# mcahny/vps

Hardware: AMD Instinct MI355X
Metric: frames/sec FuseTrack 1024x2048 (higher is better)
Workload: dtype f32-grade: f16x3 split operands (fp16 pair with scaled residual, 22 significand bits) on MFMA, f32 accumulate

## Files before the change

### vps_amd/csrc/conv_h8.hip

```cpp
#include "conv_common.h"

namespace {

template <int MODE, int KH, int KW>
__global__ __launch_bounds__(512, 2)
void conv_mfma_h8_kernel(const vps_conv_desc d, const int tiles_m, const int tiles_n, const int chunks_per_split) {
    constexpr int TM = 2, TN = 2, WAVES_N = 2, BN = 128;
    constexpr int NTAP = KH * KW;
    constexpr int HW = 32 + KW - 1, HH = 8 + KH - 1;
    constexpr int HROWS = HH * HW;
    constexpr int NLD = (HROWS + 63) / 64;
    typedef Split<MODE> SM;
    typedef typename SM::elem elem_t;
    typedef vec8<elem_t> x8;
    typedef vec4<elem_t> x4;
    constexpr int NSA = SM::NSA, NSB = SM::NSB;
    constexpr int PLANE = NLD * 64 * LDS_LDH;
    constexpr int ABUF = NSA * PLANE;
    constexpr int NLB = NSB;
    constexpr int NFRAG = NLB * 2 * (BN / 32);
    constexpr int BBUF = NFRAG * 512;
    static_assert((NFRAG * 64) % 512 == 0, "whole 16-byte chunks per thread");
    constexpr int NBL = NFRAG * 64 / 512;
    static_assert(2 * (ABUF + BBUF) * 2 <= 160 * 1024, "LDS budget of the CU");

    __shared__ __attribute__((aligned(16))) elem_t As[2 * ABUF];
    __shared__ __attribute__((aligned(16))) elem_t Bs[2 * BBUF];

    const int t = threadIdx.x;
    int swz = xcd_swizzle(blockIdx.x, gridDim.x);
    int tile_n, tile_m, cls, split;
    decode_tile(d, swz, tiles_n, tiles_m, tile_n, tile_m, cls, split);

    const int py = cls / d.os_x, px = cls - py * d.os_x;
    const int H = d.H, W = d.W, cin_pad = d.cin_pad;
    const int tiles_x = (d.Qw + 31) >> 5, tiles_y = (d.Qh + 7) >> 3;
    const int tx = tile_m % tiles_x, tq = tile_m / tiles_x;
    const int ty = tq % tiles_y, n = tq / tiles_y;
    const int iy_org = ty * 8 - d.pad_y[py], ix_org = tx * 32 - d.pad_x[px];

    const int k4 = t & 7;
    const int r0 = t >> 3;
    const int chunk0 = split * chunks_per_split;
    const int nchunks = min(chunks_per_split, d.kpad / (BK * NTAP) - chunk0);
    const int nsteps = nchunks * NTAP;

    const int lane = t & 63;
    const int wave = __builtin_amdgcn_readfirstlane(t >> 6);
    const int wm = wave / WAVES_N, wn = wave - wm * WAVES_N;
    const int nbt = d.cout_pad >> 5, kst = d.kpad >> 4;
    const size_t wplane = (size_t)d.nclass * nbt * kst * 512;
    const __amdgpu_buffer_rsrc_t wrsrc = make_rsrc(d.w_split, (unsigned)(wplane * NSB * sizeof(elem_t)));
    const unsigned wbase = (unsigned)((((size_t)(cls * nbt + tile_n * (BN / 32)) * kst + 2 * (size_t)chunk0 * NTAP) * 512) * sizeof(elem_t));
    const __amdgpu_buffer_rsrc_t arsrc = make_rsrc(d.in, (unsigned)((size_t)d.N * H * W * d.in_ld * sizeof(float)));
    const unsigned ld4 = (unsigned)d.in_ld * 4u;

    f32x4 areg[NLD];
    int achunk = chunk0;
    x8 breg[NBL];
    float amax = 0.f;

    unsigned hoff[NLD];
#pragma unroll
    for (int i = 0; i < NLD; ++i) {
        const int hp = r0 + 64 * i;
        const int hy = hp / HW, hx = hp - hy * HW;
        const int iy = iy_org + hy, ix = ix_org + hx;
        const bool ok = hp < HROWS && (unsigned)iy < (unsigned)H && (unsigned)ix < (unsigned)W;
        hoff[i] = ok ? (unsigned)((n * H + iy) * W + ix) * ld4 + (unsigned)(d.in_coff + k4 * 4) * 4u : 0xFFFFFFF0u;
    }

    auto load_A = [&]() {
        const bool kv = achunk * BK + k4 * 4 < cin_pad;
        const unsigned coff = (unsigned)achunk * (BK * 4u);
        ++achunk;
#pragma unroll
        for (int i = 0; i < NLD; ++i)
            areg[i] = buffer_load16<f32x4>(arsrc, (kv && hoff[i] != 0xFFFFFFF0u) ? hoff[i] + coff : 0xFFFFFFF0u, 0u);
    };
    auto store_A = [&](int i, int buf) {
        x4 sp[NSA];
        split_act<MODE>(areg[i], sp, amax);
        const int row = r0 + 64 * i;
#pragma unroll
        for (int p = 0; p < NSA; ++p)
            *reinterpret_cast<x4*>(&As[buf * ABUF + p * PLANE + row * LDS_LDH + (((k4 >> 1) ^ lds_swz(row)) << 3) + ((k4 & 1) << 2)]) = sp[p];
    };
    auto load_B = [&](int step) {
#pragma unroll
        for (int j = 0; j < NBL; ++j) {
            const int f = __builtin_amdgcn_readfirstlane((t + 512 * j) >> 6), bcol = f % (BN / 32), pm = f / (BN / 32);
            breg[j] = buffer_load16<x8>(wrsrc, (unsigned)lane * 16u,
                                        wbase + (unsigned)(((size_t)(pm >> 1) * wplane + ((size_t)bcol * kst + 2 * step + (pm & 1)) * 512) * sizeof(elem_t)));
        }
    };
    auto store_B = [&](int buf) {
#pragma unroll
        for (int j = 0; j < NBL; ++j) *reinterpret_cast<x8*>(&Bs[buf * BBUF + (t + 512 * j) * 8]) = breg[j];
    };

    int hbase[TM];
#pragma unroll
    for (int a = 0; a < TM; ++a) hbase[a] = (wm * TM + a) * HW + (lane & 31);
    x8 af[2][NSA][TM];
    auto read_A = [&](int m, int buf, int toff) {
#pragma unroll
        for (int a = 0; a < TM; ++a) {
            const int hrow = hbase[a] + toff;
            const int off = buf * ABUF + hrow * LDS_LDH + (((2 * m + (lane >> 5)) ^ lds_swz(hrow)) << 3);
#pragma unroll
            for (int p = 0; p < NSA; ++p) af[m][p][a] = *reinterpret_cast<const x8*>(&As[off + p * PLANE]);
        }
    };
    x8 bcur[2][NSB][TN];
    auto read_B = [&](int m, int buf) {
#pragma unroll
        for (int p = 0; p < NLB; ++p)
#pragma unroll
            for (int b = 0; b < TN; ++b)
                bcur[m][p][b] = *reinterpret_cast<const x8*>(&Bs[buf * BBUF + (((p * 2 + m) * (BN / 32)) + wn * TN + b) * 512 + lane * 8]);
        if constexpr (NLB < NSB) {
#pragma unroll
            for (int b = 0; b < TN; ++b) bcur[m][2][b] = derive_weight_plane<MODE>(bcur[m][0][b]);
        }
    };

    f32x16 acc[TM][TN];
#pragma unroll
    for (int a = 0; a < TM; ++a)
#pragma unroll
        for (int b = 0; b < TN; ++b)
#pragma unroll
            for (int r = 0; r < 16; ++r) acc[a][b][r] = 0.f;

    load_A();
    load_B(0);
#pragma unroll
    for (int i = 0; i < NLD; ++i) store_A(i, 0);
    store_B(0);
    load_A();
    __syncthreads();

    constexpr int NT = SM::NT;
    constexpr int NMF = 2 * NT * TM * TN;
    constexpr int SPT = (NLD + NTAP - 2) / (NTAP - 1);
    constexpr int NW = SPT + 3;

    for (int chunk = 0; chunk < nchunks; ++chunk) {
        const int cur = chunk & 1;
#pragma unroll
        for (int tp = 0; tp < NTAP; ++tp) {
            const int step = chunk * NTAP + tp;
            const int bb = step & 1;
            const int bstep = min(step + 1, nsteps - 1);
            const int toff = (tp / KW) * HW + (tp % KW);
            read_A(0, cur, toff);
            read_B(0, bb);
            __builtin_amdgcn_sched_barrier(0);

            auto work = [&](const int w) {
                if (w == 0) load_B(bstep);
                else if (w == 1) { read_A(1, cur, toff); read_B(1, bb); }
                else if (w < SPT + 2) {
                    const int si = w - 2;
                    if (tp < NTAP - 1) {
                        const int row = tp * SPT + si;
                        if (row < NLD) store_A(row, cur ^ 1);
                    } else if (si == 0) load_A();
                } else store_B(bb ^ 1);
            };

            int mf = 0;
#pragma unroll
            for (int m = 0; m < 2; ++m)
#pragma unroll
                for (int q = 0; q < NT; ++q)
#pragma unroll
                    for (int a = 0; a < TM; ++a)
#pragma unroll
                        for (int b = 0; b < TN; ++b) {
                            acc[a][b] = split_mfma<MODE>(bcur[m][SM::PB[q]][b], af[m][SM::PA[q]][a], acc[a][b]);
                            ++mf;
#pragma unroll
                            for (int w = 0; w < NW; ++w) {
                                const int pos = ((w + 1) * NMF) / (NW + 1);
                                if (mf == (pos < 1 ? 1 : pos)) {
                                    __builtin_amdgcn_sched_barrier(0);
                                    work(w);
                                    __builtin_amdgcn_sched_barrier(0);
                                }
                            }
                        }
            __syncthreads();
        }
    }
    report_range<MODE>(d, amax);
    conv_epilogue<TM, TN, BN, true, 5>(d, acc, tiles_m * 256, tile_m, tile_n, cls, split, py, px, wm, wn, lane, (cls * tiles_m + tile_m) * tiles_n + tile_n);
}

struct S2Tap { int ph, j, i, idx, t, nt; };
constexpr int s2_taps_1d(int K, int a) { return (K - a + 1) / 2; }
constexpr S2Tap s2_tap(int K, int ts) {
    int base = 0;
    for (int ph = 0; ph < 4; ++ph) {
        const int a = ph >> 1, b = ph & 1, J = s2_taps_1d(K, a), I = s2_taps_1d(K, b);
        if (ts < base + J * I) {
            const int t = ts - base, j = t / I, i = t - j * I;
            return S2Tap{ph, j, i, (2 * j + a) * K + 2 * i + b, t, J * I};
        }
        base += J * I;
    }
    return S2Tap{0, 0, 0, 0, 0, 1};
}
template <int N, typename F>
__device__ __forceinline__ void static_for(F&& f) {
    if constexpr (N > 0) {
        static_for<N - 1>(f);
        f(std::integral_constant<int, N - 1>{});
    }
}

template <int MODE, int K, int BN = 128>
__global__ __launch_bounds__(512, 2)
void conv_mfma_h8s2_kernel(const vps_conv_desc d, const int tiles_m, const int tiles_n, const int chunks_per_split) {
    static_assert(BN == 128 || BN == 64, "two column waves of 64 or 32 columns");
    constexpr int TM = 2, TN = BN / 64, WAVES_N = 2;
    constexpr int NTAP = K * K;
    constexpr int J0 = s2_taps_1d(K, 0);
    constexpr int HW = 32 + J0 - 1, HH = 8 + J0 - 1;
    constexpr int HROWS = HH * HW;
    constexpr int NLD = (HROWS + 63) / 64;
    typedef Split<MODE> SM;
    typedef typename SM::elem elem_t;
    typedef vec8<elem_t> x8;
    typedef vec4<elem_t> x4;
    constexpr int NSA = SM::NSA, NSB = SM::NSB;
    constexpr int PLANE = NLD * 64 * LDS_LDH;
    constexpr int ABUF = NSA * PLANE;
    constexpr int NLB = NSB;
    constexpr int NFRAG = NLB * 2 * (BN / 32);
    constexpr int NBL = (NFRAG * 64 + 511) / 512;
    constexpr bool WHOLE = (NFRAG * 64) % 512 == 0;
    constexpr int BBUF = NBL * 512 * 8;
    static_assert(2 * (ABUF + BBUF) * 2 <= 160 * 1024, "LDS budget of the CU");

    __shared__ __attribute__((aligned(16))) elem_t As[2 * ABUF];
    __shared__ __attribute__((aligned(16))) elem_t Bs[2 * BBUF];

    const int t = threadIdx.x;
    const int swz = xcd_swizzle(blockIdx.x, gridDim.x);
    int tile_n, tile_m, cls, split;
    decode_tile(d, swz, tiles_n, tiles_m, tile_n, tile_m, cls, split);

    const int H = d.H, W = d.W, cin_pad = d.cin_pad;
    const int tiles_x = (d.Qw + 31) >> 5, tiles_y = (d.Qh + 7) >> 3;
    const int tx = tile_m % tiles_x, tq = tile_m / tiles_x;
    const int ty = tq % tiles_y, n = tq / tiles_y;
    const int iy_org = ty * 16 - d.pad_y[0], ix_org = tx * 64 - d.pad_x[0];

    const int k4 = t & 7;
    const int r0 = t >> 3;
    const int chunk0 = split * chunks_per_split;
    const int nchunks = min(chunks_per_split, d.kpad / (BK * NTAP) - chunk0);

    const int lane = t & 63;
    const int wave = __builtin_amdgcn_readfirstlane(t >> 6);
    const int wm = wave / WAVES_N, wn = wave - wm * WAVES_N;
    const int nbt = d.cout_pad >> 5, kst = d.kpad >> 4;
    const size_t wplane = (size_t)nbt * kst * 512;
    const __amdgpu_buffer_rsrc_t wrsrc = make_rsrc(d.w_split, (unsigned)(wplane * NSB * sizeof(elem_t)));
    const unsigned wbase = (unsigned)((((size_t)(tile_n * (BN / 32)) * kst + 2 * (size_t)chunk0 * NTAP) * 512) * sizeof(elem_t));
    const __amdgpu_buffer_rsrc_t arsrc = make_rsrc(d.in, (unsigned)((size_t)d.N * H * W * d.in_ld * sizeof(float)));
    const unsigned ld4 = (unsigned)d.in_ld * 4u;

    f32x4 areg[NLD];
    int achunk = chunk0, aph = 0;
    x8 breg[NBL];
    float amax = 0.f;

    auto load_A = [&]() {
        const int a = aph >> 1, b = aph & 1;
        const int rows = 8 + ((K - a + 1) >> 1) - 1, cols = 32 + ((K - b + 1) >> 1) - 1;
        const int cic = achunk * BK + k4 * 4;
        const bool kv = cic < cin_pad;
        const unsigned coff = (unsigned)(d.in_coff + cic) * 4u;
        if (++aph == 4) { aph = 0; ++achunk; }
#pragma unroll
        for (int i = 0; i < NLD; ++i) {
            const int hp = r0 + 64 * i;
            const int hy = hp / HW, hx = hp - hy * HW;
            const int iy = iy_org + a + 2 * hy, ix = ix_org + b + 2 * hx;
            const bool ok = kv && hy < rows && hx < cols && (unsigned)iy < (unsigned)H && (unsigned)ix < (unsigned)W;
            areg[i] = buffer_load16<f32x4>(arsrc, ok ? (unsigned)((n * H + iy) * W + ix) * ld4 + coff : 0xFFFFFFF0u, 0u);
        }
    };
    auto store_A = [&](int i, int buf) {
        x4 sp[NSA];
        split_act<MODE>(areg[i], sp, amax);
        const int row = r0 + 64 * i;
#pragma unroll
        for (int p = 0; p < NSA; ++p)
            *reinterpret_cast<x4*>(&As[buf * ABUF + p * PLANE + row * LDS_LDH + (((k4 >> 1) ^ lds_swz(row)) << 3) + ((k4 & 1) << 2)]) = sp[p];
    };
    auto load_B = [&](int wstep) {
#pragma unroll
        for (int j = 0; j < NBL; ++j) {
            const int fr = __builtin_amdgcn_readfirstlane((t + 512 * j) >> 6), f = WHOLE ? fr : min(fr, NFRAG - 1);
            const int bcol = f % (BN / 32), pm = f / (BN / 32);
            breg[j] = buffer_load16<x8>(wrsrc, (unsigned)lane * 16u,
                                        wbase + (unsigned)(((size_t)(pm >> 1) * wplane + ((size_t)bcol * kst + 2 * wstep + (pm & 1)) * 512) * sizeof(elem_t)));
        }
    };
    auto store_B = [&](int buf) {
#pragma unroll
        for (int j = 0; j < NBL; ++j)
            *reinterpret_cast<x8*>(&Bs[buf * BBUF + (t + 512 * j) * 8]) = breg[j];
    };

    int hbase[TM];
#pragma unroll
    for (int a = 0; a < TM; ++a) hbase[a] = (wm * TM + a) * HW + (lane & 31);
    x8 af[2][NSA][TM];
    auto read_A = [&](int m, int buf, int toff) {
#pragma unroll
        for (int a = 0; a < TM; ++a) {
            const int hrow = hbase[a] + toff;
            const int off = buf * ABUF + hrow * LDS_LDH + (((2 * m + (lane >> 5)) ^ lds_swz(hrow)) << 3);
#pragma unroll
            for (int p = 0; p < NSA; ++p) af[m][p][a] = *reinterpret_cast<const x8*>(&As[off + p * PLANE]);
        }
    };
    x8 bcur[2][NSB][TN];
    auto read_B = [&](int m, int buf) {
#pragma unroll
        for (int p = 0; p < NLB; ++p)
#pragma unroll
            for (int b = 0; b < TN; ++b)
                bcur[m][p][b] = *reinterpret_cast<const x8*>(&Bs[buf * BBUF + (((p * 2 + m) * (BN / 32)) + wn * TN + b) * 512 + lane * 8]);
        if constexpr (NLB < NSB) {
#pragma unroll
            for (int b = 0; b < TN; ++b) bcur[m][2][b] = derive_weight_plane<MODE>(bcur[m][0][b]);
        }
    };

    f32x16 acc[TM][TN];
#pragma unroll
    for (int a = 0; a < TM; ++a)
#pragma unroll
        for (int b = 0; b < TN; ++b)
#pragma unroll
            for (int r = 0; r < 16; ++r) acc[a][b][r] = 0.f;

    load_A();
    load_B(s2_tap(K, 0).idx);
#pragma unroll
    for (int i = 0; i < NLD; ++i) store_A(i, 0);
    store_B(0);
    load_A();
    __syncthreads();

    constexpr int NT = SM::NT;
    constexpr int NMF = 2 * NT * TM * TN;

    for (int chunk = 0; chunk < nchunks; ++chunk) {
        static_for<NTAP>([&](auto ts_tag) {
            constexpr int TS = decltype(ts_tag)::value;
            constexpr S2Tap tp = s2_tap(K, TS);
            constexpr S2Tap nx = s2_tap(K, (TS + 1) % NTAP);
            constexpr int cur = tp.ph & 1;
            constexpr bool last_of_phase = tp.t == tp.nt - 1;
            constexpr int SPT = (NLD + tp.nt - 1) / tp.nt;
            constexpr int NW = 3 + SPT + (last_of_phase ? 1 : 0);
            const int step = chunk * NTAP + TS;
            const int bb = step & 1;
            const int wnext = (TS + 1 < NTAP ? chunk : min(chunk + 1, nchunks - 1)) * NTAP + nx.idx;
            constexpr int toff = tp.j * HW + tp.i;
            read_A(0, cur, toff);
            read_B(0, bb);
            __builtin_amdgcn_sched_barrier(0);

            auto work = [&](const int w) {
                if (w == 0) load_B(wnext);
                else if (w == 1) { read_A(1, cur, toff); read_B(1, bb); }
                else if (w < SPT + 2) {
                    const int row = tp.t * SPT + (w - 2);
                    if (row < NLD) store_A(row, cur ^ 1);
                } else if (last_of_phase && w == SPT + 2) load_A();
                else store_B(bb ^ 1);
            };

            int mf = 0;
#pragma unroll
            for (int m = 0; m < 2; ++m)
#pragma unroll
                for (int q = 0; q < NT; ++q)
#pragma unroll
                    for (int a = 0; a < TM; ++a)
#pragma unroll
                        for (int b = 0; b < TN; ++b) {
                            acc[a][b] = split_mfma<MODE>(bcur[m][SM::PB[q]][b], af[m][SM::PA[q]][a], acc[a][b]);
                            ++mf;
#pragma unroll
                            for (int w = 0; w < NW; ++w) {
                                const int pos = ((w + 1) * NMF) / (NW + 1);
                                if (mf == (pos < 1 ? 1 : pos)) {
                                    __builtin_amdgcn_sched_barrier(0);
                                    work(w);
                                    __builtin_amdgcn_sched_barrier(0);
                                }
                            }
                        }
            __syncthreads();
        });
    }
    report_range<MODE>(d, amax);
    conv_epilogue<TM, TN, BN, true, 5>(d, acc, tiles_m * 256, tile_m, tile_n, cls, split, 0, 0, wm, wn, lane, (cls * tiles_m + tile_m) * tiles_n + tile_n);
}

}

int vpsi_launch_conv_h8p(const vps_conv_desc& d, int tiles_m8, int tiles_n, int chunks_per_split, long nblk8, hipStream_t s);

__attribute__((visibility("hidden")))
void vpsi_launch_conv_h8(const vps_conv_desc& d, int tiles_m8, int tiles_n, int chunks_per_split, long nblk8, hipStream_t s) {
    if (vpsi_launch_conv_h8p(d, tiles_m8, tiles_n, chunks_per_split, nblk8, s)) return;
#define VPS_H8_LAUNCH(MODE, K)                                                                                                   \
    hipLaunchKernelGGL((conv_mfma_h8_kernel<MODE, K, K>), dim3((unsigned)nblk8), dim3(512), 0, s, d, tiles_m8, tiles_n, chunks_per_split)
    if (d.prec == VPS_PREC_BF16) { if (d.KH == 3) VPS_H8_LAUNCH(VPS_PREC_BF16, 3); else VPS_H8_LAUNCH(VPS_PREC_BF16, 2); }
    else if (d.prec == VPS_PREC_BF16X3) { if (d.KH == 3) VPS_H8_LAUNCH(VPS_PREC_BF16X3, 3); else VPS_H8_LAUNCH(VPS_PREC_BF16X3, 2); }
    else { if (d.KH == 3) VPS_H8_LAUNCH(VPS_PREC_F16X3, 3); else VPS_H8_LAUNCH(VPS_PREC_F16X3, 2); }
#undef VPS_H8_LAUNCH
}

__attribute__((visibility("hidden")))
void vpsi_launch_conv_h8s2(const vps_conv_desc& d, int tiles_m8, int tiles_n, int chunks_per_split, long nblk8, int bn, hipStream_t s) {
#define VPS_H8S2_LAUNCH(MODE, K)                                                                                                 \
    do {                                                                                                                         \
        if (bn == 64) hipLaunchKernelGGL((conv_mfma_h8s2_kernel<MODE, K, 64>), dim3((unsigned)nblk8), dim3(512), 0, s, d, tiles_m8, tiles_n, chunks_per_split); \
        else hipLaunchKernelGGL((conv_mfma_h8s2_kernel<MODE, K, 128>), dim3((unsigned)nblk8), dim3(512), 0, s, d, tiles_m8, tiles_n, chunks_per_split);         \
    } while (0)
    if (d.prec == VPS_PREC_BF16) { if (d.KH == 3) VPS_H8S2_LAUNCH(VPS_PREC_BF16, 3); else VPS_H8S2_LAUNCH(VPS_PREC_BF16, 5); }
    else if (d.prec == VPS_PREC_BF16X3) { if (d.KH == 3) VPS_H8S2_LAUNCH(VPS_PREC_BF16X3, 3); else VPS_H8S2_LAUNCH(VPS_PREC_BF16X3, 5); }
    else { if (d.KH == 3) VPS_H8S2_LAUNCH(VPS_PREC_F16X3, 3); else VPS_H8S2_LAUNCH(VPS_PREC_F16X3, 5); }
#undef VPS_H8S2_LAUNCH
}
```

Before: 56.47.

## Add wide-N 3x3 f16x3 conv kernel with register-staged activations

Adds a new conv kernel for 3x3 f16x3 convolutions with cout divisible by 256. It uses a 256-wide N tile with a 2x4 wave layout and TM=4, so each activation halo tile is reused across twice as many output channels. Activations are loaded into registers early and written into the second LDS buffer across the first taps, weights are DMA'd directly into LDS with buffer_load_lds, and the third weight plane is derived in registers rather than stored. The kernel is used by default when its shape conditions hold, can be turned off with VPS_H8W=0, and raises register and LDS pressure per block.

Result: faster. 57.06, median of 6 (+1.1%).

```diff
diff --git a/vps_amd/csrc/conv_h8.hip b/vps_amd/csrc/conv_h8.hip
--- a/vps_amd/csrc/conv_h8.hip
+++ b/vps_amd/csrc/conv_h8.hip
@@ -420,9 +420,11 @@
 }
 
 int vpsi_launch_conv_h8p(const vps_conv_desc& d, int tiles_m8, int tiles_n, int chunks_per_split, long nblk8, hipStream_t s);
+int vpsi_launch_conv_h8w(const vps_conv_desc& d, int tiles_m8, int chunks_per_split, hipStream_t s);
 
 __attribute__((visibility("hidden")))
 void vpsi_launch_conv_h8(const vps_conv_desc& d, int tiles_m8, int tiles_n, int chunks_per_split, long nblk8, hipStream_t s) {
+    if (vpsi_launch_conv_h8w(d, tiles_m8, chunks_per_split, s)) return;
     if (vpsi_launch_conv_h8p(d, tiles_m8, tiles_n, chunks_per_split, nblk8, s)) return;
 #define VPS_H8_LAUNCH(MODE, K)                                                                                                   \
     hipLaunchKernelGGL((conv_mfma_h8_kernel<MODE, K, K>), dim3((unsigned)nblk8), dim3(512), 0, s, d, tiles_m8, tiles_n, chunks_per_split)
diff --git a/vps_amd/csrc/conv_h8w.hip b/vps_amd/csrc/conv_h8w.hip
--- /dev/null
+++ b/vps_amd/csrc/conv_h8w.hip
@@ -0,0 +1,231 @@
+#include "conv_common.h"
+
+namespace {
+
+template <int N, typename F>
+__device__ __forceinline__ void static_for_w(F&& f) {
+    if constexpr (N > 0) {
+        static_for_w<N - 1>(f);
+        f(std::integral_constant<int, N - 1>{});
+    }
+}
+
+template <int N>
+__device__ __forceinline__ void wait_vm_lgkm0() {
+    static_assert(N >= 0 && N < 64, "vmcnt range");
+    asm volatile("s_waitcnt vmcnt(%0) lgkmcnt(0)" ::"n"(N) : "memory");
+}
+
+__global__ __launch_bounds__(512, 2)
+void conv_mfma_h8w_kernel(const vps_conv_desc d, const int tiles_m, const int tiles_n, const int chunks_per_split) {
+    constexpr int MODE = VPS_PREC_F16X3;
+    constexpr int KH = 3, KW = 3;
+    constexpr int TM = 4, TN = 2, WAVES_N = 4, BN = 256;
+    constexpr int NTAP = KH * KW;
+    constexpr int HW = 32 + KW - 1, HH = 8 + KH - 1;
+    constexpr int HROWS = HH * HW;
+    constexpr int NLD = (HROWS + 63) / 64;
+    typedef Split<MODE> SM;
+    typedef typename SM::elem elem_t;
+    typedef vec8<elem_t> x8;
+    typedef vec4<elem_t> x4;
+    constexpr int NSA = SM::NSA, NLB = SM::NLB;
+    static_assert(NSA == 2 && NLB == 2 && SM::NSB == 3 && SM::NT == 3, "f16x3: two activation planes, two stored weight planes");
+    constexpr int PLANE = HROWS * LDS_LDH;
+    constexpr int ABUF = NSA * PLANE;
+    constexpr int NFRAG = NLB * 2 * (BN / 32);
+    constexpr int BBUF = NFRAG * 512;
+    constexpr int NDMA = NFRAG / 8;
+    constexpr int STG = (NLD + 1) / 2;
+    constexpr int LDA = NTAP - 2;
+    static_assert(STG <= LDA, "rows staged before the registers are reloaded");
+    static_assert((2 * ABUF + 2 * BBUF) * 2 + 16 <= 160 * 1024, "LDS budget of the CU");
+
+    __shared__ __attribute__((aligned(16))) elem_t lds[2 * ABUF + 2 * BBUF + 8];
+    elem_t* const As = lds;
+    elem_t* const Bs = lds + 2 * ABUF;
+
+    const int t = threadIdx.x;
+    const int swz = xcd_swizzle(blockIdx.x, gridDim.x);
+    int tile_n, tile_m, cls, split;
+    decode_tile(d, swz, tiles_n, tiles_m, tile_n, tile_m, cls, split);
+
+    const int py = cls / d.os_x, px = cls - py * d.os_x;
+    const int H = d.H, W = d.W, cin_pad = d.cin_pad;
+    const int tiles_x = (d.Qw + 31) >> 5, tiles_y = (d.Qh + 7) >> 3;
+    const int tx = tile_m % tiles_x, tq = tile_m / tiles_x;
+    const int ty = tq % tiles_y, n = tq / tiles_y;
+    const int iy_org = ty * 8 - d.pad_y[py], ix_org = tx * 32 - d.pad_x[px];
+
+    const int k4 = t & 7;
+    const int r0 = t >> 3;
+    const int chunk0 = split * chunks_per_split;
+    const int nchunks = min(chunks_per_split, d.kpad / (BK * NTAP) - chunk0);
+    const int nsteps = nchunks * NTAP;
+
+    const int lane = t & 63;
+    const int wave = __builtin_amdgcn_readfirstlane(t >> 6);
+    const int wm = wave / WAVES_N, wn = wave - wm * WAVES_N;
+    const int nbt = d.cout_pad >> 5, kst = d.kpad >> 4;
+    const size_t wplane = (size_t)d.nclass * nbt * kst * 512;
+    const __amdgpu_buffer_rsrc_t wrsrc = make_rsrc(d.w_split, (unsigned)(wplane * SM::NSB * sizeof(elem_t)));
+    const unsigned wbase = (unsigned)((((size_t)(cls * nbt + tile_n * (BN / 32)) * kst + 2 * (size_t)chunk0 * NTAP) * 512) * sizeof(elem_t));
+    const __amdgpu_buffer_rsrc_t arsrc = make_rsrc(d.in, (unsigned)((size_t)d.N * H * W * d.in_ld * sizeof(float)));
+    const unsigned ld4 = (unsigned)d.in_ld * 4u;
+
+    f32x4 areg[NLD];
+    int achunk = chunk0;
+    float amax = 0.f;
+
+    unsigned hoff[NLD];
+#pragma unroll
+    for (int i = 0; i < NLD; ++i) {
+        const int hp = r0 + 64 * i;
+        const int hy = hp / HW, hx = hp - hy * HW;
+        const int iy = iy_org + hy, ix = ix_org + hx;
+        const bool ok = hp < HROWS && (unsigned)iy < (unsigned)H && (unsigned)ix < (unsigned)W;
+        hoff[i] = ok ? (unsigned)((n * H + iy) * W + ix) * ld4 + (unsigned)(d.in_coff + k4 * 4) * 4u : 0xFFFFFFF0u;
+    }
+
+    auto load_A = [&]() {
+        const bool kv = achunk * BK + k4 * 4 < cin_pad;
+        const unsigned coff = (unsigned)achunk * (BK * 4u);
+        ++achunk;
+#pragma unroll
+        for (int i = 0; i < NLD; ++i)
+            areg[i] = buffer_load16<f32x4>(arsrc, (kv && hoff[i] != 0xFFFFFFF0u) ? hoff[i] + coff : 0xFFFFFFF0u, 0u);
+    };
+    auto store_A = [&](const int i, const int buf) {
+        x4 sp[NSA];
+        split_act<MODE>(areg[i], sp, amax);
+        const int row = r0 + 64 * i;
+        if (row < HROWS) {
+#pragma unroll
+            for (int p = 0; p < NSA; ++p)
+                *reinterpret_cast<x4*>(&As[buf * ABUF + p * PLANE + row * LDS_LDH + (((k4 >> 1) ^ lds_swz(row)) << 3) + ((k4 & 1) << 2)]) = sp[p];
+        }
+    };
+    auto dma_B = [&](const int step, const int slot) {
+        const int sc = min(step, nsteps - 1);
+#pragma unroll
+        for (int j = 0; j < NDMA; ++j) {
+            const int p = j >> 1, slab = j & 1;
+            const unsigned soff = wbase + (unsigned)(((size_t)p * wplane + ((size_t)wave * kst + 2 * sc + slab) * 512) * sizeof(elem_t));
+            __builtin_amdgcn_raw_ptr_buffer_load_lds(wrsrc, (__attribute__((address_space(3))) void*)&Bs[slot * BBUF + (j * 8 + wave) * 512],
+                                                     16, (unsigned)lane * 16u, soff, 0, 0);
+        }
+    };
+
+    int hbase[TM];
+#pragma unroll
+    for (int a = 0; a < TM; ++a) hbase[a] = (wm * TM + a) * HW + (lane & 31);
+    x8 af[2][NSA];
+    x8 bf[2][NLB][TN];
+    auto read_A = [&](x8 (&dst)[NSA], const int m, const int a, const int abuf, const int toff) {
+        const int hrow = hbase[a] + toff;
+#pragma unroll
+        for (int p = 0; p < NSA; ++p)
+            dst[p] = *reinterpret_cast<const x8*>(&As[abuf * ABUF + p * PLANE + hrow * LDS_LDH + (((2 * m + (lane >> 5)) ^ lds_swz(hrow)) << 3)]);
+    };
+    auto read_B = [&](x8 (&dst)[NLB][TN], const int m, const int slot) {
+#pragma unroll
+        for (int p = 0; p < NLB; ++p)
+#pragma unroll
+            for (int b = 0; b < TN; ++b)
+                dst[p][b] = *reinterpret_cast<const x8*>(&Bs[slot * BBUF + (((p * 2 + m) * (BN / 32)) + wn * TN + b) * 512 + lane * 8]);
+    };
+
+    f32x16 acc[TM][TN];
+#pragma unroll
+    for (int a = 0; a < TM; ++a)
+#pragma unroll
+        for (int b = 0; b < TN; ++b)
+#pragma unroll
+            for (int r = 0; r < 16; ++r) acc[a][b][r] = 0.f;
+
+    load_A();
+    dma_B(0, 0);
+#pragma unroll
+    for (int i = 0; i < NLD; ++i) store_A(i, 0);
+    load_A();
+    wait_vm_lgkm0<NLD>();
+    __builtin_amdgcn_sched_barrier(0);
+    __builtin_amdgcn_s_barrier();
+    __builtin_amdgcn_sched_barrier(0);
+
+    auto tap = [&](const int chunk, auto tp_tag) {
+        constexpr int tp = decltype(tp_tag)::value;
+        constexpr int toff = (tp / KW) * HW + (tp % KW);
+        const int cur = chunk & 1;
+        const int step = chunk * NTAP + tp;
+        const int slot = step & 1;
+#pragma unroll
+        for (int a = 0; a < TM; ++a) asm volatile("" : "+v"(hbase[a]));
+        read_B(bf[0], 0, slot);
+        read_A(af[0], 0, 0, cur, toff);
+        __builtin_amdgcn_sched_barrier(0);
+        if constexpr (tp < STG) {
+            store_A(2 * tp, cur ^ 1);
+            if (2 * tp + 1 < NLD) store_A(2 * tp + 1, cur ^ 1);
+        }
+        dma_B(step + 1, slot ^ 1);
+        if constexpr (tp == LDA) load_A();
+        __builtin_amdgcn_sched_barrier(0);
+        x8 bd[TN];
+#pragma unroll
+        for (int u = 0; u < 2 * TM; ++u) {
+            const int m = u / TM, a = u % TM;
+            if (u + 1 < 2 * TM) {
+                read_A(af[(u + 1) & 1], (u + 1) / TM, (u + 1) % TM, cur, toff);
+                if ((u + 1) % TM == 0) read_B(bf[1], 1, slot);
+            }
+            __builtin_amdgcn_sched_barrier(0);
+            if (a == 0) {
+#pragma unroll
+                for (int b = 0; b < TN; ++b) bd[b] = derive_weight_plane<MODE>(bf[m][0][b]);
+            }
+#pragma unroll
+            for (int q = 0; q < SM::NT; ++q)
+#pragma unroll
+                for (int b = 0; b < TN; ++b) {
+                    const x8 bw = SM::PB[q] == 2 ? bd[b] : bf[m][SM::PB[q]][b];
+                    acc[a][b] = split_mfma<MODE>(bw, af[u & 1][SM::PA[q]], acc[a][b]);
+                }
+            __builtin_amdgcn_sched_barrier(0);
+        }
+        if constexpr (tp == LDA) wait_vm_lgkm0<NLD>();
+        else wait_vm_lgkm0<0>();
+        __builtin_amdgcn_sched_barrier(0);
+        __builtin_amdgcn_s_barrier();
+        __builtin_amdgcn_sched_barrier(0);
+    };
+
+    for (int chunk = 0; chunk < nchunks; ++chunk)
+        static_for_w<NTAP>([&](auto tpc) { tap(chunk, tpc); });
+
+    report_range<MODE>(d, amax);
+#pragma unroll
+    for (int h = 0; h < 2; ++h)
+#pragma unroll
+        for (int b = 0; b < TN; ++b) {
+            f32x16 part[2][1] = {{acc[2 * h][b]}, {acc[2 * h + 1][b]}};
+            conv_epilogue<2, 1, BN, true, 5, false, true>(d, part, tiles_m * 256, tile_m, tile_n, cls, split, py, px, 2 * wm + h, 2 * wn + b, lane,
+                                                          (cls * tiles_m + tile_m) * tiles_n + tile_n, reinterpret_cast<int*>(&lds[2 * ABUF + 2 * BBUF]));
+        }
+}
+
+}
+
+__attribute__((visibility("hidden")))
+int vpsi_launch_conv_h8w(const vps_conv_desc& d, int tiles_m8, int chunks_per_split, hipStream_t s) {
+    const char* const e = getenv("VPS_H8W");
+    if (e && atoi(e) == 0) return 0;
+    if (d.prec != VPS_PREC_F16X3 || d.KH != 3 || d.KW != 3) return 0;
+    if (d.ksplit != 1 || chunks_per_split < d.kpad / (BK * 9)) return 0;
+    if (d.cout_pad % 256) return 0;
+    const int tiles_n = d.cout_pad / 256;
+    const long nblk = (long)tiles_m8 * tiles_n * d.nclass;
+    if (nblk < 256 || nblk > 0x7fffffffL) return 0;
+    hipLaunchKernelGGL(conv_mfma_h8w_kernel, dim3((unsigned)nblk), dim3(512), 0, s, d, tiles_m8, tiles_n, chunks_per_split);
+    return 1;
+}
```
